# autonomousvision/unimatch

Measured on NVIDIA H100. Metric: image-pairs/sec @480x832 gmflow-scale2-refine6; EPE vs reference, higher is better.
Workload: dtype fp32

## Files before the change

unimatch_b200/csrc/um_conv_tc.cu:

```cuda
#include <stdlib.h>

#include "um_common.cuh"
#include "um_tc.cuh"

namespace um {

using namespace tc;

namespace {

constexpr int TW = 16, TH = 8;
__host__ __device__ constexpr int stages_for(int bn) { return bn >= 96 ? 2 : 3; }
constexpr int NTHREADS = 288;
constexpr int PRODUCER = 8;
constexpr uint32_t A_BYTES = 2 * 16384;
constexpr uint32_t STAGING_UNIT = 16384;
constexpr uint32_t STAGING_BYTES = 2 * STAGING_UNIT;
constexpr uint32_t TAIL_BYTES = 256 + 2048;
__host__ __device__ constexpr uint32_t acc_bytes(int bn) { return (bn < 32 ? 32 : bn) * 128 * 4; }
__host__ __device__ constexpr uint32_t conv_smem_bytes(int bn) {
  return stages_for(bn) * (A_BYTES + 2 * bn * 128) + acc_bytes(bn) + STAGING_BYTES + TAIL_BYTES;
}

struct ConvParams {
  int B, H, W, tiles_x, tiles_y;
  int nsrc, cin_p[2];
  int KH, KW, PH, PW, stride;
  int cout, cout_p;
  const float* bias;
  int mode, act;
  float* out_f32; long long ld_f32; int off_f32;
  __half* out_split; int cp_split, off_split; long long plane_split;
  const float* aux0; long long ld_aux0;
  const float* aux1; long long ld_aux1;
  const float* gamma; const float* beta;
  const float* pre; long long ld_pre;
  int ntiles, tiles_n;
  __half* win_dst; long long win_plane;
  int win_c0, win_c1, win_lp;
  long long win_tokens, win_L;
  Geom win_g;
};

__device__ __forceinline__ float sigmoid_fast(float y) { return __fdividef(1.0f, 1.0f + __expf(-y)); }
__device__ __forceinline__ float tanh_fast(float y) { return 1.0f - __fdividef(2.0f, 1.0f + __expf(2.0f * y)); }
__device__ __forceinline__ uint32_t pack_h2(__half a, __half b) {
  return (uint32_t)__half_as_ushort(a) | ((uint32_t)__half_as_ushort(b) << 16);
}

__device__ __forceinline__ void load_acc32(const float* accs, int r, int c0, float* v) {
  const float* row = accs + (c0 >> 5) * 4096 + r * 32;
#pragma unroll
  for (int i = 0; i < 8; ++i) {
    const float4 x = *reinterpret_cast<const float4*>(row + ((i ^ (r & 7)) << 2));
    v[4 * i] = x.x; v[4 * i + 1] = x.y; v[4 * i + 2] = x.z; v[4 * i + 3] = x.w;
  }
}

template <int BN, int G, int MODE, int ACT, bool WIN = false>
__global__ void __launch_bounds__(NTHREADS, 1)
conv_tc_kernel(const __grid_constant__ CUtensorMap map_a0, const __grid_constant__ CUtensorMap map_a1,
               const __grid_constant__ CUtensorMap map_w, const __grid_constant__ CUtensorMap map_of,
               const __grid_constant__ CUtensorMap map_os, ConvParams p) {
  static_assert(BN == 16 || BN == 64 || BN == 96 || BN == 128, "tile widths 16, 64, 96, 128");
  constexpr int NSB = 1;
  constexpr uint32_t B_BYTES = 2 * BN * 128;
  constexpr uint32_t STAGE_BYTES = A_BYTES + B_BYTES;
  constexpr int STAGES = stages_for(BN);
  constexpr uint32_t ACC_BYTES = acc_bytes(BN);
  extern __shared__ __align__(1024) uint8_t smem[];
  float* accs = reinterpret_cast<float*>(smem + STAGES * STAGE_BYTES);
  float* stage_buf = reinterpret_cast<float*>(smem + STAGES * STAGE_BYTES + ACC_BYTES);
  uint64_t* bars = reinterpret_cast<uint64_t*>(smem + STAGES * STAGE_BYTES + ACC_BYTES + STAGING_BYTES);
  uint64_t* full = bars;
  uint64_t* empty = bars + STAGES;
  float* coef = reinterpret_cast<float*>(reinterpret_cast<uint8_t*>(bars) + 256);
  const int mode = MODE >= 0 ? MODE : p.mode;
  const int act = ACT >= 0 ? ACT : p.act;

  const int warp = threadIdx.x >> 5, lane = threadIdx.x & 31;
  const int taps = p.KH * p.KW;
  int nk = 0;
  for (int s = 0; s < p.nsrc; ++s) nk += taps * (p.cin_p[s] >> 6);

  const int cid = (int)blockIdx.x;
  const int ncid = (int)gridDim.x;

  if (threadIdx.x == 0) {
    for (int i = 0; i < STAGES; ++i) { mbar_init(full + i, 1); mbar_init(empty + i, 8); }
    fence_barrier_init();
  }
  if (warp == PRODUCER && lane == 0) {
    tma_prefetch_desc(&map_a0); tma_prefetch_desc(&map_w);
    if (p.nsrc > 1) tma_prefetch_desc(&map_a1);
  }
  __syncthreads();

  if (warp == PRODUCER) {
    int it = 0;
    for (int t = cid; t < p.ntiles; t += ncid) {
      const int n0 = (t % p.tiles_n) * BN;
      int tile = t / p.tiles_n;
      const int x0 = (tile % p.tiles_x) * TW; tile /= p.tiles_x;
      const int y0 = (tile % p.tiles_y) * TH;
      const int b = tile / p.tiles_y;
      const int chunks0 = p.cin_p[0] >> 6;
      const int nk0 = taps * chunks0;
      const int rot = (int)((unsigned)cid % (unsigned)nk);
      for (int kk = 0; kk < nk; ++kk, ++it) {
        int k = kk + rot; if (k >= nk) k -= nk;
        const int sidx = (k >= nk0) ? 1 : 0;
        const int kl = sidx ? k - nk0 : k;
        const int chunks = sidx ? (p.cin_p[1] >> 6) : chunks0;
        const int tap = kl / chunks, kc = kl - tap * chunks;
        const int ky = tap / p.KW, kx = tap - ky * p.KW;
        const CUtensorMap* ma = sidx ? &map_a1 : &map_a0;
        const int st = it % STAGES;
        mbar_wait_inline(empty + st, ((it / STAGES) & 1) ^ 1);
        uint8_t* sa = smem + st * STAGE_BYTES;
        uint8_t* sb = sa + A_BYTES;
        const int kcol = (sidx ? taps * p.cin_p[0] : 0) + tap * p.cin_p[sidx] + kc * 64;
        if (elect_one()) {
          mbar_arrive_expect_tx(full + st, STAGE_BYTES);
#pragma unroll
          for (int part = 0; part < 2; ++part) {
            tma_load_4d(sa + part * 16384, ma, full + st, kc * 64, x0 * p.stride + kx - p.PW, y0 * p.stride + ky - p.PH, part * p.B + b);
            tma_load_2d(sb + part * (BN * 128), &map_w, full + st, kcol, part * p.cout_p + n0);
          }
        }
        __syncwarp();
      }
    }
  } else {
    const int quarter = warp & 3;
    const int grp = warp >> 2;
    const int r = quarter * 32 + lane;
    const int eg = (warp & 3) * 32 + lane;
    const int frow = grp * 64 + quarter * 16 + (lane >> 2);
    const int fcol = 2 * (lane & 3);
    const bool leader = eg == 0;
    int sctr = 0;
    auto group_sync = [&]() { asm volatile("bar.sync %0, 128;" ::"r"(1 + grp) : "memory"); };
    auto all_sync = [&]() { asm volatile("bar.sync 3, 256;" ::: "memory"); };
    if (mode == UM_CONV_LN && grp == 0) { coef[256 + eg] = __ldg(p.gamma + eg); coef[384 + eg] = __ldg(p.beta + eg); }
    int lt = 0, it = 0;
    for (int t = cid; t < p.ntiles; t += ncid, ++lt) {
      float acc[BN / 2], part[BN / 2];
      for (int k = 0; k < nk; ++k, ++it) {
        const int st = it % STAGES;
        mbar_wait_inline(full + st, (it / STAGES) & 1);
        const uint32_t a_base = smem_u32(smem + st * STAGE_BYTES) + grp * 8192;
        const uint32_t b_base = smem_u32(smem + st * STAGE_BYTES) + A_BYTES;
        const int pa[3] = {1, 0, 0}, pb[3] = {0, 1, 0};
        if (G > 1) fence_acc(part); else fence_acc(acc);
        wgmma_fence();
#pragma unroll
        for (int c = 0; c < 3; ++c)
#pragma unroll
          for (int ks = 0; ks < 4; ++ks) {
            const uint64_t da = desc_kmajor(a_base + pa[c] * 16384 + ks * 32);
            const uint64_t db = desc_kmajor(b_base + pb[c] * (BN * 128) + ks * 32);
            if (G > 1) wgmma_ss<BN>(part, da, db, (c | ks) != 0);
            else wgmma_ss<BN>(acc, da, db, k > 0 || (c | ks) != 0);
          }
        wgmma_commit();
        wgmma_wait<0>();
        if (G > 1) fence_acc(part); else fence_acc(acc);
        __syncwarp();
        if (lane == 0) mbar_arrive(empty + st);
        if (G > 1) {
#pragma unroll
          for (int i = 0; i < BN / 2; ++i) acc[i] = k ? acc[i] + part[i] : part[i];
        }
      }
      all_sync();
#pragma unroll
      for (int j = 0; j < BN / 8; ++j) {
        const int col = 8 * j + fcol;
        float* chunk = accs + (col >> 5) * 4096;
#pragma unroll
        for (int h = 0; h < 2; ++h) {
          const int row = frow + 8 * h;
          *reinterpret_cast<float2*>(chunk + row * 32 + ((((col & 31) >> 2) ^ (row & 7)) << 2) + (col & 3)) =
              make_float2(acc[4 * j + 2 * h], acc[4 * j + 2 * h + 1]);
        }
      }
      all_sync();

      const int n0 = (t % p.tiles_n) * BN;
      int tile = t / p.tiles_n;
      const int x0 = (tile % p.tiles_x) * TW; tile /= p.tiles_x;
      const int y0 = (tile % p.tiles_y) * TH;
      const int b = tile / p.tiles_y;
      const long long pix_r = ((long long)b * p.H + (y0 + (r >> 4))) * p.W + x0 + (r & 15);
      const bool valid_r = (y0 + (r >> 4) < p.H) && (x0 + (r & 15) < p.W);

      auto emit = [&](const float (&v)[32], int co_out, bool to_f32, bool to_split, bool to_win = false) {
        if (WIN && to_win) {
          uint8_t* sbs = reinterpret_cast<uint8_t*>(stage_buf + (grp * NSB + sctr % NSB) * 4096);
          ++sctr;
          if (leader) bulk_wait_read<NSB - 1>();
          group_sync();
#pragma unroll
          for (int i = 0; i < 4; ++i) {
            uint32_t hw[4], lw[4];
#pragma unroll
            for (int e = 0; e < 4; ++e) split_f16x2(v[8 * i + 2 * e], v[8 * i + 2 * e + 1], &hw[e], &lw[e]);
            const int off = r * 64 + ((i ^ ((r >> 1) & 3)) << 4);
            *reinterpret_cast<uint4*>(sbs + off) = make_uint4(hw[0], hw[1], hw[2], hw[3]);
            *reinterpret_cast<uint4*>(sbs + 8192 + off) = make_uint4(lw[0], lw[1], lw[2], lw[3]);
          }
          group_sync();
          const int wc = co_out - p.win_c0;
          __half* obase = p.win_dst + (long long)(wc >> 7) * 2 * p.win_plane + (wc & 127);
          const int* rowdst = reinterpret_cast<const int*>(coef + 256) + (lt & 1) * 128;
          const int piece = eg & 3;
#pragma unroll
          for (int itr = 0; itr < 4; ++itr) {
            const int row = itr * 32 + (eg >> 2);
            const int drow = rowdst[row];
            if (drow < 0) continue;
            const int soff = row * 64 + ((piece ^ ((row >> 1) & 3)) << 4);
            const uint4 hv = *reinterpret_cast<const uint4*>(sbs + soff);
            const uint4 lv = *reinterpret_cast<const uint4*>(sbs + 8192 + soff);
            __half* d = obase + (long long)drow * 128 + piece * 8;
            *reinterpret_cast<uint4*>(d) = hv;
            *reinterpret_cast<uint4*>(d + p.win_plane) = lv;
          }
          return;
        }
        if (to_f32) {
          float* my_stage = stage_buf + (grp * NSB + sctr % NSB) * 4096;
          ++sctr;
          if (leader) bulk_wait_read<NSB - 1>();
          group_sync();
#pragma unroll
          for (int i = 0; i < 8; ++i)
            *reinterpret_cast<float4*>(my_stage + r * 32 + ((i ^ (r & 7)) << 2)) = make_float4(v[4 * i], v[4 * i + 1], v[4 * i + 2], v[4 * i + 3]);
          fence_proxy_async();
          group_sync();
          if (leader) { tma_store_4d(&map_of, my_stage, co_out, x0, y0, b); bulk_commit(); }
        }
        if (to_split) {
          uint8_t* sbs = reinterpret_cast<uint8_t*>(stage_buf + (grp * NSB + sctr % NSB) * 4096);
          ++sctr;
          if (leader) bulk_wait_read<NSB - 1>();
          group_sync();
#pragma unroll
          for (int i = 0; i < 4; ++i) {
            uint32_t hw[4], lw[4];
#pragma unroll
            for (int e = 0; e < 4; ++e) split_f16x2(v[8 * i + 2 * e], v[8 * i + 2 * e + 1], &hw[e], &lw[e]);
            const int off = r * 64 + ((i ^ ((r >> 1) & 3)) << 4);
            *reinterpret_cast<uint4*>(sbs + off) = make_uint4(hw[0], hw[1], hw[2], hw[3]);
            *reinterpret_cast<uint4*>(sbs + 8192 + off) = make_uint4(lw[0], lw[1], lw[2], lw[3]);
          }
          fence_proxy_async();
          group_sync();
          if (leader) {
            tma_store_4d(&map_os, sbs, co_out, x0, y0, b);
            tma_store_4d(&map_os, sbs + 8192, co_out, x0, y0, p.B + b);
            bulk_commit();
          }
        }
      };

      if constexpr (BN == 128) {
        if (mode == UM_CONV_LN) {
          const int ca = grp * 32, cb = 64 + grp * 32;
          float a0[32], a1[32];
          const bool need_a = valid_r && p.aux0;
          if (need_a) {
            const float4* pa = reinterpret_cast<const float4*>(p.aux0 + pix_r * p.ld_aux0 + ca);
            const float4* pb = reinterpret_cast<const float4*>(p.aux0 + pix_r * p.ld_aux0 + cb);
#pragma unroll
            for (int i = 0; i < 8; ++i) {
              const float4 t4 = __ldg(pa + i), u4 = __ldg(pb + i);
              a0[4 * i] = t4.x; a0[4 * i + 1] = t4.y; a0[4 * i + 2] = t4.z; a0[4 * i + 3] = t4.w;
              a1[4 * i] = u4.x; a1[4 * i + 1] = u4.y; a1[4 * i + 2] = u4.z; a1[4 * i + 3] = u4.w;
            }
          }
          float v0[32], v1[32];
          load_acc32(accs, r, ca, v0);
          load_acc32(accs, r, cb, v1);
          float* xs = coef;
          float sum = 0.f;
#pragma unroll
          for (int i = 0; i < 32; ++i) sum += v0[i];
#pragma unroll
          for (int i = 0; i < 32; ++i) sum += v1[i];
          xs[grp * 128 + r] = sum;
          all_sync();
          const float mean = (xs[r] + xs[128 + r]) * (1.0f / 128.0f);
          all_sync();
          float sq = 0.f;
#pragma unroll
          for (int i = 0; i < 32; ++i) { const float dd = v0[i] - mean; sq = fmaf(dd, dd, sq); }
#pragma unroll
          for (int i = 0; i < 32; ++i) { const float dd = v1[i] - mean; sq = fmaf(dd, dd, sq); }
          xs[grp * 128 + r] = sq;
          all_sync();
          const float rstd = rsqrtf((xs[r] + xs[128 + r]) * (1.0f / 128.0f) + 1e-5f);
          const float4* g4a = reinterpret_cast<const float4*>(coef + 256 + ca);
          const float4* b4a = reinterpret_cast<const float4*>(coef + 384 + ca);
          const float4* g4b = reinterpret_cast<const float4*>(coef + 256 + cb);
          const float4* b4b = reinterpret_cast<const float4*>(coef + 384 + cb);
#pragma unroll
          for (int i = 0; i < 8; ++i) {
            const float4 ga = g4a[i], ba = b4a[i], gb = g4b[i], bb = b4b[i];
            v0[4 * i] = (v0[4 * i] - mean) * rstd * ga.x + ba.x;             v1[4 * i] = (v1[4 * i] - mean) * rstd * gb.x + bb.x;
            v0[4 * i + 1] = (v0[4 * i + 1] - mean) * rstd * ga.y + ba.y;     v1[4 * i + 1] = (v1[4 * i + 1] - mean) * rstd * gb.y + bb.y;
            v0[4 * i + 2] = (v0[4 * i + 2] - mean) * rstd * ga.z + ba.z;     v1[4 * i + 2] = (v1[4 * i + 2] - mean) * rstd * gb.z + bb.z;
            v0[4 * i + 3] = (v0[4 * i + 3] - mean) * rstd * ga.w + ba.w;     v1[4 * i + 3] = (v1[4 * i + 3] - mean) * rstd * gb.w + bb.w;
          }
          if (need_a) {
#pragma unroll
            for (int i = 0; i < 32; ++i) { v0[i] += a0[i]; v1[i] += a1[i]; }
          }
          emit(v0, ca, p.out_f32 != nullptr, p.out_split != nullptr);
          emit(v1, cb, p.out_f32 != nullptr, p.out_split != nullptr);
          continue;
        }
      }

      float* sbias = coef + (lt & 1) * 128;
      if (grp == 0) {
        for (int i = eg; i < BN; i += 128) sbias[i] = (p.bias && n0 + i < p.cout) ? __ldg(p.bias + n0 + i) : 0.f;
        if (WIN) {
          const int yy = y0 + (eg >> 4), xx = x0 + (eg & 15);
          const long long token = ((long long)b * p.H + yy) * p.W + xx;
          int drow = -1;
          if (yy < p.H && xx < p.W && token < p.win_tokens) {
            const Geom& g = p.win_g;
            const int n = (int)(token / p.win_L);
            const int t = (int)(token - (long long)n * p.win_L);
            const int ty = t / g.w, tx = t - ty * g.w;
            int yr = ty - g.sh; if (yr < 0) yr += g.h;
            int xr = tx - g.sw; if (xr < 0) xr += g.w;
            const int wy = yr / g.wh, wx = xr / g.ww;
            drow = (n * g.nwin + wy * g.kw + wx) * p.win_lp + (yr - wy * g.wh) * g.ww + (xr - wx * g.ww);
          }
          reinterpret_cast<int*>(coef + 256)[(lt & 1) * 128 + eg] = drow;
        }
      }
      all_sync();
      if (grp * 32 >= BN) continue;

      constexpr int CH = BN < 32 ? BN : 32;
#pragma unroll 1
      for (int c0 = grp * 32; c0 < BN; c0 += 64) {
        const int co0 = n0 + c0;
        const bool live = co0 < p.cout;
        bool to_f32 = p.out_f32 != nullptr, to_split = p.out_split != nullptr;
        int co_out = co0;
        if (mode == UM_CONV_GRU_ZR) {
          to_f32 = co0 < 128; to_split = co0 >= 128;
          if (co0 >= 128) co_out = co0 - 128;
        }
        bool to_win = false;
        if (WIN && co0 >= p.win_c0 && co0 < p.win_c1) { to_win = true; to_f32 = to_split = false; }
        float ax[32], bx[32];
        const bool need_a = live && valid_r && p.aux0 && (mode == UM_CONV_GRU_Q || (mode == UM_CONV_GRU_ZR && co0 >= 128));
        const bool need_b = live && valid_r && mode == UM_CONV_GRU_Q;
        if (need_a) {
          const float4* ap = reinterpret_cast<const float4*>(p.aux0 + pix_r * p.ld_aux0 + (mode == UM_CONV_GRU_ZR ? co0 - 128 : co0));
#pragma unroll
          for (int i = 0; i < 8; ++i) { const float4 t4 = __ldg(ap + i); ax[4 * i] = t4.x; ax[4 * i + 1] = t4.y; ax[4 * i + 2] = t4.z; ax[4 * i + 3] = t4.w; }
        }
        if (need_b) {
          const float4* bp = reinterpret_cast<const float4*>(p.aux1 + pix_r * p.ld_aux1 + co0);
#pragma unroll
          for (int i = 0; i < 8; ++i) { const float4 t4 = __ldg(bp + i); bx[4 * i] = t4.x; bx[4 * i + 1] = t4.y; bx[4 * i + 2] = t4.z; bx[4 * i + 3] = t4.w; }
        }
        float px[32];
        const bool need_p = live && valid_r && p.pre;
        if (need_p) {
          const float4* pp = reinterpret_cast<const float4*>(p.pre + pix_r * p.ld_pre + co0);
#pragma unroll
          for (int i = 0; i < 8; ++i) { const float4 t4 = __ldg(pp + i); px[4 * i] = t4.x; px[4 * i + 1] = t4.y; px[4 * i + 2] = t4.z; px[4 * i + 3] = t4.w; }
        }
        float v[32];
        load_acc32(accs, r, c0, v);
        if (!live) continue;
        if (p.bias) {
          const float4* s4 = reinterpret_cast<const float4*>(sbias + c0);
#pragma unroll
          for (int i = 0; i < CH / 4; ++i) {
            const float4 bb = s4[i];
            v[4 * i] += bb.x; v[4 * i + 1] += bb.y; v[4 * i + 2] += bb.z; v[4 * i + 3] += bb.w;
          }
        }
        if (need_p) {
#pragma unroll
          for (int i = 0; i < CH; ++i) v[i] += px[i];
        }
        if (mode == UM_CONV_GRU_ZR) {
#pragma unroll
          for (int i = 0; i < CH; ++i) v[i] = sigmoid_fast(v[i]);
          if (need_a) {
#pragma unroll
            for (int i = 0; i < CH; ++i) v[i] *= ax[i];
          }
        } else if (mode == UM_CONV_GRU_Q) {
          if (need_b) {
#pragma unroll
            for (int i = 0; i < CH; ++i) v[i] = (1.0f - bx[i]) * ax[i] + bx[i] * tanh_fast(v[i]);
          }
        } else if (act == UM_ACT_RELU) {
#pragma unroll
          for (int i = 0; i < CH; ++i) v[i] = fmaxf(v[i], 0.f);
        } else if (act == UM_ACT_TANH) {
#pragma unroll
          for (int i = 0; i < CH; ++i) v[i] = tanh_fast(v[i]);
        } else if (act == UM_ACT_SIGMOID) {
#pragma unroll
          for (int i = 0; i < CH; ++i) v[i] = sigmoid_fast(v[i]);
        } else if (act == UM_ACT_GELU) {
#pragma unroll
          for (int i = 0; i < CH; ++i) v[i] = act_gelu(v[i]);
        }
        if constexpr (BN >= 32) {
          emit(v, co_out, to_f32, to_split, to_win);
        } else {
          const int nvalid = min(CH, p.cout - co0);
          float* sb = stage_buf + grp * NSB * 4096;
          group_sync();
#pragma unroll
          for (int i = 0; i < CH / 4; ++i)
            *reinterpret_cast<float4*>(sb + r * 32 + ((i ^ (r & 7)) << 2)) = make_float4(v[4 * i], v[4 * i + 1], v[4 * i + 2], v[4 * i + 3]);
          group_sync();
          if (to_f32) {
#pragma unroll 1
            for (int itr = 0; itr < 8; ++itr) {
              const int row = itr * 16 + (eg >> 3), piece = eg & 7;
              const int yy = y0 + (row >> 4), xx = x0 + (row & 15);
              if (yy >= p.H || xx >= p.W || piece * 4 >= nvalid) continue;
              const float4 val = *reinterpret_cast<const float4*>(sb + row * 32 + ((piece ^ (row & 7)) << 2));
              float* dst = p.out_f32 + (((long long)b * p.H + yy) * p.W + xx) * p.ld_f32 + p.off_f32 + co_out + piece * 4;
              const float e[4] = {val.x, val.y, val.z, val.w};
              for (int k = 0; k < 4; ++k) if (piece * 4 + k < nvalid) dst[k] = e[k];
            }
          }
          if (to_split) {
#pragma unroll 1
            for (int itr = 0; itr < 4; ++itr) {
              const int row = itr * 32 + (eg >> 2), piece = eg & 3;
              const int yy = y0 + (row >> 4), xx = x0 + (row & 15);
              if (yy >= p.H || xx >= p.W || piece * 8 >= nvalid) continue;
              const float4 a4 = *reinterpret_cast<const float4*>(sb + row * 32 + (((2 * piece) ^ (row & 7)) << 2));
              const float4 c4 = *reinterpret_cast<const float4*>(sb + row * 32 + (((2 * piece + 1) ^ (row & 7)) << 2));
              const float e[8] = {a4.x, a4.y, a4.z, a4.w, c4.x, c4.y, c4.z, c4.w};
              __half* dh = p.out_split + (((long long)b * p.H + yy) * p.W + xx) * p.cp_split + p.off_split + co_out + piece * 8;
              __half* dl = dh + p.plane_split;
              for (int k = 0; k < 8; ++k)
                if (piece * 8 + k < nvalid) { __half h0, l0; split_f16(e[k], &h0, &l0); dh[k] = h0; dl[k] = l0; }
            }
          }
        }
      }
    }
    if (leader) bulk_wait_all();
  }
}

template <int VEC>
__global__ void __launch_bounds__(256) split_planes_kernel(const float* __restrict__ src, long long ld, int C,
                                                           __half* __restrict__ dst, int cp, int off, long long plane,
                                                           long long rows) {
  const int per_row = C / VEC;
  const long long i = (long long)blockIdx.x * blockDim.x + threadIdx.x;
  if (i >= rows * per_row) return;
  const long long row = i / per_row;
  const int c = (int)(i - row * per_row) * VEC;
  if (VEC == 4) {
    const float4 x = __ldg(reinterpret_cast<const float4*>(src + row * ld + c));
    __half h[4], l[4];
    split_f16(x.x, &h[0], &l[0]); split_f16(x.y, &h[1], &l[1]); split_f16(x.z, &h[2], &l[2]); split_f16(x.w, &h[3], &l[3]);
    *reinterpret_cast<uint2*>(dst + row * cp + off + c) = make_uint2(pack_h2(h[0], h[1]), pack_h2(h[2], h[3]));
    *reinterpret_cast<uint2*>(dst + plane + row * cp + off + c) = make_uint2(pack_h2(l[0], l[1]), pack_h2(l[2], l[3]));
  } else {
    __half h, l;
    split_f16(__ldg(src + row * ld + c), &h, &l);
    dst[row * cp + off + c] = h;
    dst[plane + row * cp + off + c] = l;
  }
}

}

int make_map_4d_f16(CUtensorMap* map, const void* base, uint64_t cp, uint64_t W, uint64_t H, uint64_t NB, uint32_t stride,
                    uint64_t plane_elems) {
  PFN_encodeTiled enc = get_encode_tiled();
  if (!enc) { set_error("cuTensorMapEncodeTiled unavailable"); return UM_ECUDA; }
  cuuint64_t dims[4] = {cp, W, H, NB};
  cuuint64_t strides[3] = {cp * 2, cp * W * 2, (plane_elems ? plane_elems : cp * W * H) * 2};
  cuuint32_t box[4] = {64, 16 * stride, 8 * stride, 1};
  cuuint32_t estr[4] = {1, stride, stride, 1};
  CUresult r = enc(map, CU_TENSOR_MAP_DATA_TYPE_FLOAT16, 4, const_cast<void*>(base), dims, strides, box, estr,
                   CU_TENSOR_MAP_INTERLEAVE_NONE, CU_TENSOR_MAP_SWIZZLE_128B, CU_TENSOR_MAP_L2_PROMOTION_L2_128B,
                   CU_TENSOR_MAP_FLOAT_OOB_FILL_NONE);
  if (r != CUDA_SUCCESS) { set_error("cuTensorMapEncodeTiled(4d) failed (%d)", (int)r); return UM_ECUDA; }
  return UM_OK;
}

int make_map_out(CUtensorMap* map, void* base, int elem_bytes, uint64_t cout, uint64_t ld, uint64_t W, uint64_t H, uint64_t N,
                 uint64_t plane_elems) {
  PFN_encodeTiled enc = get_encode_tiled();
  if (!enc) { set_error("cuTensorMapEncodeTiled unavailable"); return UM_ECUDA; }
  cuuint64_t dims[4] = {cout, W, H, N};
  cuuint64_t strides[3] = {ld * elem_bytes, ld * W * elem_bytes, (plane_elems ? plane_elems : ld * W * H) * elem_bytes};
  cuuint32_t box[4] = {32, 16, 8, 1};
  cuuint32_t estr[4] = {1, 1, 1, 1};
  CUresult r = enc(map, elem_bytes == 4 ? CU_TENSOR_MAP_DATA_TYPE_FLOAT32 : CU_TENSOR_MAP_DATA_TYPE_FLOAT16, 4, base, dims,
                   strides, box, estr, CU_TENSOR_MAP_INTERLEAVE_NONE,
                   elem_bytes == 4 ? CU_TENSOR_MAP_SWIZZLE_128B : CU_TENSOR_MAP_SWIZZLE_64B,
                   CU_TENSOR_MAP_L2_PROMOTION_NONE, CU_TENSOR_MAP_FLOAT_OOB_FILL_NONE);
  if (r != CUDA_SUCCESS) { set_error("cuTensorMapEncodeTiled(out) failed (%d)", (int)r); return UM_ECUDA; }
  return UM_OK;
}

namespace {

template <int BN, int G, int MODE, int ACT, bool WIN = false>
int launch_conv(const CUtensorMap& m0, const CUtensorMap& m1, const CUtensorMap& mw, const CUtensorMap& mof,
                const CUtensorMap& mos, const ConvParams& p, cudaStream_t st) {
  constexpr uint32_t smem = conv_smem_bytes(BN);
  static_assert(smem <= 232448, "shared memory budget");
  static PerDeviceBytes configured;
  if (int rc = ensure_smem(configured, conv_tc_kernel<BN, G, MODE, ACT, WIN>, smem, "conv_tc")) return rc;
// ... 161 lines not shown
```

unimatch_b200/csrc/um_tc.cuh:

```cuda
#pragma once
#include <cuda.h>
#include <cuda_fp16.h>
#include <cuda_runtime.h>
#include <stdint.h>

namespace um {
namespace tc {

__device__ __forceinline__ uint32_t smem_u32(const void* p) { return (uint32_t)__cvta_generic_to_shared(p); }

__device__ __forceinline__ bool elect_one() {
  uint32_t pred = 0;
  asm volatile(
      "{\n\t.reg .pred P;\n\telect.sync _|P, 0xffffffff;\n\tselp.u32 %0, 1, 0, P;\n\t}\n"
      : "=r"(pred));
  return pred != 0;
}

__device__ __forceinline__ void mbar_init(uint64_t* bar, uint32_t count) {
  asm volatile("mbarrier.init.shared::cta.b64 [%0], %1;" ::"r"(smem_u32(bar)), "r"(count));
}
__device__ __forceinline__ void fence_barrier_init() { asm volatile("fence.mbarrier_init.release.cluster;" ::: "memory"); }
__device__ __forceinline__ void fence_proxy_async() { asm volatile("fence.proxy.async.shared::cta;" ::: "memory"); }
__device__ __forceinline__ void mbar_arrive(uint64_t* bar) {
  asm volatile("mbarrier.arrive.shared::cta.b64 _, [%0];" ::"r"(smem_u32(bar)) : "memory");
}
__device__ __forceinline__ void mbar_arrive_expect_tx(uint64_t* bar, uint32_t bytes) {
  asm volatile("mbarrier.arrive.expect_tx.shared::cta.b64 _, [%0], %1;" ::"r"(smem_u32(bar)), "r"(bytes) : "memory");
}
__device__ __forceinline__ bool mbar_try_wait(uint64_t* bar, uint32_t parity) {
  uint32_t ok;
  asm volatile(
      "{\n\t.reg .pred P;\n\tmbarrier.try_wait.parity.shared::cta.b64 P, [%1], %2;\n\tselp.u32 %0, 1, 0, P;\n\t}\n"
      : "=r"(ok)
      : "r"(smem_u32(bar)), "r"(parity)
      : "memory");
  return ok != 0;
}
static __device__ __noinline__ void mbar_wait_slow(uint64_t* bar, uint32_t parity) {
#pragma unroll 1
  for (uint32_t i = 0; i < (1u << 22); ++i)
    if (mbar_try_wait(bar, parity)) return;
  printf("um::tc mbarrier timeout: block (%d,%d,%d) thread %d bar %p parity %u\n", blockIdx.x, blockIdx.y, blockIdx.z,
         threadIdx.x, (void*)bar, parity);
  __trap();
}
__device__ __forceinline__ void mbar_wait(uint64_t* bar, uint32_t parity) {
  if (!mbar_try_wait(bar, parity)) mbar_wait_slow(bar, parity);
}
__device__ __forceinline__ void mbar_wait_inline(uint64_t* bar, uint32_t parity) {
#pragma unroll 1
  for (uint32_t i = 0; !mbar_try_wait(bar, parity); ++i)
    if (i == (1u << 22)) __trap();
}

__device__ __forceinline__ void tma_prefetch_desc(const CUtensorMap* m) {
  asm volatile("prefetch.tensormap [%0];" ::"l"(reinterpret_cast<uint64_t>(m)) : "memory");
}
__device__ __forceinline__ void tma_load_2d(void* dst, const CUtensorMap* m, uint64_t* bar, int c0, int c1) {
  asm volatile(
      "cp.async.bulk.tensor.2d.shared::cluster.global.mbarrier::complete_tx::bytes [%0], [%1, {%3, %4}], [%2];"
      ::"r"(smem_u32(dst)), "l"(reinterpret_cast<uint64_t>(m)), "r"(smem_u32(bar)), "r"(c0), "r"(c1)
      : "memory");
}
__device__ __forceinline__ void tma_load_4d(void* dst, const CUtensorMap* m, uint64_t* bar, int c0, int c1, int c2, int c3) {
  asm volatile(
      "cp.async.bulk.tensor.4d.shared::cluster.global.mbarrier::complete_tx::bytes [%0], [%1, {%3, %4, %5, %6}], [%2];"
      ::"r"(smem_u32(dst)), "l"(reinterpret_cast<uint64_t>(m)), "r"(smem_u32(bar)), "r"(c0), "r"(c1), "r"(c2), "r"(c3)
      : "memory");
}

__device__ __forceinline__ void tma_store_4d(const CUtensorMap* m, const void* src, int c0, int c1, int c2, int c3) {
  asm volatile("cp.async.bulk.tensor.4d.global.shared::cta.bulk_group [%0, {%2, %3, %4, %5}], [%1];"
               ::"l"(reinterpret_cast<uint64_t>(m)), "r"(smem_u32(src)), "r"(c0), "r"(c1), "r"(c2), "r"(c3)
               : "memory");
}
__device__ __forceinline__ void bulk_commit() { asm volatile("cp.async.bulk.commit_group;" ::: "memory"); }
template <int N>
__device__ __forceinline__ void bulk_wait_read() { asm volatile("cp.async.bulk.wait_group.read %0;" ::"n"(N) : "memory"); }
__device__ __forceinline__ void bulk_wait_all() { asm volatile("cp.async.bulk.wait_group 0;" ::: "memory"); }

__device__ __forceinline__ uint64_t smem_desc_sw128(uint32_t saddr, uint32_t lbo_bytes, uint32_t sbo_bytes) {
  uint64_t d = 0;
  d |= (uint64_t)((saddr & 0x3FFFF) >> 4);
  d |= (uint64_t)((lbo_bytes >> 4) & 0x3FFF) << 16;
  d |= (uint64_t)((sbo_bytes >> 4) & 0x3FFF) << 32;
  d |= (uint64_t)1 << 62;
  return d;
}
__device__ __forceinline__ uint64_t desc_kmajor(uint32_t saddr) { return smem_desc_sw128(saddr, 16, 1024); }
__device__ __forceinline__ uint64_t desc_mnmajor(uint32_t saddr, uint32_t mn_group_stride) {
  return smem_desc_sw128(saddr, mn_group_stride, 1024);
}

__device__ __forceinline__ void wgmma_fence() { asm volatile("wgmma.fence.sync.aligned;" ::: "memory"); }
__device__ __forceinline__ void wgmma_commit() { asm volatile("wgmma.commit_group.sync.aligned;" ::: "memory"); }
template <int N>
__device__ __forceinline__ void wgmma_wait() { asm volatile("wgmma.wait_group.sync.aligned %0;" ::"n"(N) : "memory"); }
template <int N>
__device__ __forceinline__ void fence_acc(float (&d)[N]) {
#pragma unroll
  for (int i = 0; i < N; ++i) asm volatile("" : "+f"(d[i])::"memory");
}

template <int N>
__device__ __forceinline__ void wgmma_ss(float (&d)[N / 2], uint64_t da, uint64_t db, bool accumulate);
template <>
__device__ __forceinline__ void wgmma_ss<16>(float (&d)[8], uint64_t da, uint64_t db, bool accumulate) {
  asm volatile(
      "{\n\t.reg .pred p;\n\tsetp.ne.b32 p, %10, 0;\n\t"
      "wgmma.mma_async.sync.aligned.m64n16k16.f32.f16.f16 {%0, %1, %2, %3, %4, %5, %6, %7}, %8, %9, p, 1, 1, 0, 0;\n\t}\n"
      : "+f"(d[0]), "+f"(d[1]), "+f"(d[2]), "+f"(d[3]), "+f"(d[4]), "+f"(d[5]), "+f"(d[6]), "+f"(d[7])
      : "l"(da), "l"(db), "r"((uint32_t)accumulate));
}
template <>
__device__ __forceinline__ void wgmma_ss<64>(float (&d)[32], uint64_t da, uint64_t db, bool accumulate) {
  asm volatile(
      "{\n\t.reg .pred p;\n\tsetp.ne.b32 p, %34, 0;\n\t"
      "wgmma.mma_async.sync.aligned.m64n64k16.f32.f16.f16 {%0, %1, %2, %3, %4, %5, %6, %7, %8, %9, %10, %11, %12, %13, %14, %15, %16, %17, %18, %19, %20, %21, %22, %23, %24, %25, %26, %27, %28, %29, %30, %31}, %32, %33, p, 1, 1, 0, 0;\n\t}\n"
      : "+f"(d[0]), "+f"(d[1]), "+f"(d[2]), "+f"(d[3]), "+f"(d[4]), "+f"(d[5]), "+f"(d[6]), "+f"(d[7]), "+f"(d[8]), "+f"(d[9]), "+f"(d[10]), "+f"(d[11]), "+f"(d[12]), "+f"(d[13]), "+f"(d[14]), "+f"(d[15]), "+f"(d[16]), "+f"(d[17]), "+f"(d[18]), "+f"(d[19]), "+f"(d[20]), "+f"(d[21]), "+f"(d[22]), "+f"(d[23]), "+f"(d[24]), "+f"(d[25]), "+f"(d[26]), "+f"(d[27]), "+f"(d[28]), "+f"(d[29]), "+f"(d[30]), "+f"(d[31])
      : "l"(da), "l"(db), "r"((uint32_t)accumulate));
}
template <>
__device__ __forceinline__ void wgmma_ss<96>(float (&d)[48], uint64_t da, uint64_t db, bool accumulate) {
  asm volatile(
      "{\n\t.reg .pred p;\n\tsetp.ne.b32 p, %50, 0;\n\t"
      "wgmma.mma_async.sync.aligned.m64n96k16.f32.f16.f16 {%0, %1, %2, %3, %4, %5, %6, %7, %8, %9, %10, %11, %12, %13, %14, %15, %16, %17, %18, %19, %20, %21, %22, %23, %24, %25, %26, %27, %28, %29, %30, %31, %32, %33, %34, %35, %36, %37, %38, %39, %40, %41, %42, %43, %44, %45, %46, %47}, %48, %49, p, 1, 1, 0, 0;\n\t}\n"
      : "+f"(d[0]), "+f"(d[1]), "+f"(d[2]), "+f"(d[3]), "+f"(d[4]), "+f"(d[5]), "+f"(d[6]), "+f"(d[7]), "+f"(d[8]), "+f"(d[9]), "+f"(d[10]), "+f"(d[11]), "+f"(d[12]), "+f"(d[13]), "+f"(d[14]), "+f"(d[15]), "+f"(d[16]), "+f"(d[17]), "+f"(d[18]), "+f"(d[19]), "+f"(d[20]), "+f"(d[21]), "+f"(d[22]), "+f"(d[23]), "+f"(d[24]), "+f"(d[25]), "+f"(d[26]), "+f"(d[27]), "+f"(d[28]), "+f"(d[29]), "+f"(d[30]), "+f"(d[31]), "+f"(d[32]), "+f"(d[33]), "+f"(d[34]), "+f"(d[35]), "+f"(d[36]), "+f"(d[37]), "+f"(d[38]), "+f"(d[39]), "+f"(d[40]), "+f"(d[41]), "+f"(d[42]), "+f"(d[43]), "+f"(d[44]), "+f"(d[45]), "+f"(d[46]), "+f"(d[47])
      : "l"(da), "l"(db), "r"((uint32_t)accumulate));
}
template <>
__device__ __forceinline__ void wgmma_ss<128>(float (&d)[64], uint64_t da, uint64_t db, bool accumulate) {
  asm volatile(
      "{\n\t.reg .pred p;\n\tsetp.ne.b32 p, %66, 0;\n\t"
      "wgmma.mma_async.sync.aligned.m64n128k16.f32.f16.f16 {%0, %1, %2, %3, %4, %5, %6, %7, %8, %9, %10, %11, %12, %13, %14, %15, %16, %17, %18, %19, %20, %21, %22, %23, %24, %25, %26, %27, %28, %29, %30, %31, %32, %33, %34, %35, %36, %37, %38, %39, %40, %41, %42, %43, %44, %45, %46, %47, %48, %49, %50, %51, %52, %53, %54, %55, %56, %57, %58, %59, %60, %61, %62, %63}, %64, %65, p, 1, 1, 0, 0;\n\t}\n"
      : "+f"(d[0]), "+f"(d[1]), "+f"(d[2]), "+f"(d[3]), "+f"(d[4]), "+f"(d[5]), "+f"(d[6]), "+f"(d[7]), "+f"(d[8]), "+f"(d[9]), "+f"(d[10]), "+f"(d[11]), "+f"(d[12]), "+f"(d[13]), "+f"(d[14]), "+f"(d[15]), "+f"(d[16]), "+f"(d[17]), "+f"(d[18]), "+f"(d[19]), "+f"(d[20]), "+f"(d[21]), "+f"(d[22]), "+f"(d[23]), "+f"(d[24]), "+f"(d[25]), "+f"(d[26]), "+f"(d[27]), "+f"(d[28]), "+f"(d[29]), "+f"(d[30]), "+f"(d[31]), "+f"(d[32]), "+f"(d[33]), "+f"(d[34]), "+f"(d[35]), "+f"(d[36]), "+f"(d[37]), "+f"(d[38]), "+f"(d[39]), "+f"(d[40]), "+f"(d[41]), "+f"(d[42]), "+f"(d[43]), "+f"(d[44]), "+f"(d[45]), "+f"(d[46]), "+f"(d[47]), "+f"(d[48]), "+f"(d[49]), "+f"(d[50]), "+f"(d[51]), "+f"(d[52]), "+f"(d[53]), "+f"(d[54]), "+f"(d[55]), "+f"(d[56]), "+f"(d[57]), "+f"(d[58]), "+f"(d[59]), "+f"(d[60]), "+f"(d[61]), "+f"(d[62]), "+f"(d[63])
      : "l"(da), "l"(db), "r"((uint32_t)accumulate));
}
__device__ __forceinline__ void wgmma_rs_n128_tb(float (&d)[64], const uint32_t (&a)[4], uint64_t db, bool accumulate) {
  asm volatile(
      "{\n\t.reg .pred p;\n\tsetp.ne.b32 p, %69, 0;\n\t"
      "wgmma.mma_async.sync.aligned.m64n128k16.f32.f16.f16 {%0, %1, %2, %3, %4, %5, %6, %7, %8, %9, %10, %11, %12, %13, %14, %15, %16, %17, %18, %19, %20, %21, %22, %23, %24, %25, %26, %27, %28, %29, %30, %31, %32, %33, %34, %35, %36, %37, %38, %39, %40, %41, %42, %43, %44, %45, %46, %47, %48, %49, %50, %51, %52, %53, %54, %55, %56, %57, %58, %59, %60, %61, %62, %63}, {%64, %65, %66, %67}, %68, p, 1, 1, 1;\n\t}\n"
      : "+f"(d[0]), "+f"(d[1]), "+f"(d[2]), "+f"(d[3]), "+f"(d[4]), "+f"(d[5]), "+f"(d[6]), "+f"(d[7]), "+f"(d[8]), "+f"(d[9]), "+f"(d[10]), "+f"(d[11]), "+f"(d[12]), "+f"(d[13]), "+f"(d[14]), "+f"(d[15]), "+f"(d[16]), "+f"(d[17]), "+f"(d[18]), "+f"(d[19]), "+f"(d[20]), "+f"(d[21]), "+f"(d[22]), "+f"(d[23]), "+f"(d[24]), "+f"(d[25]), "+f"(d[26]), "+f"(d[27]), "+f"(d[28]), "+f"(d[29]), "+f"(d[30]), "+f"(d[31]), "+f"(d[32]), "+f"(d[33]), "+f"(d[34]), "+f"(d[35]), "+f"(d[36]), "+f"(d[37]), "+f"(d[38]), "+f"(d[39]), "+f"(d[40]), "+f"(d[41]), "+f"(d[42]), "+f"(d[43]), "+f"(d[44]), "+f"(d[45]), "+f"(d[46]), "+f"(d[47]), "+f"(d[48]), "+f"(d[49]), "+f"(d[50]), "+f"(d[51]), "+f"(d[52]), "+f"(d[53]), "+f"(d[54]), "+f"(d[55]), "+f"(d[56]), "+f"(d[57]), "+f"(d[58]), "+f"(d[59]), "+f"(d[60]), "+f"(d[61]), "+f"(d[62]), "+f"(d[63])
      : "r"(a[0]), "r"(a[1]), "r"(a[2]), "r"(a[3]), "l"(db), "r"((uint32_t)accumulate));
}

__device__ __forceinline__ void wgmma_rs_n64(float (&d)[32], const uint32_t (&a)[4], uint64_t db, bool accumulate) {
  asm volatile(
      "{\n\t.reg .pred p;\n\tsetp.ne.b32 p, %37, 0;\n\t"
      "wgmma.mma_async.sync.aligned.m64n64k16.f32.f16.f16 {%0, %1, %2, %3, %4, %5, %6, %7, %8, %9, %10, %11, %12, %13, %14, %15, %16, %17, %18, %19, %20, %21, %22, %23, %24, %25, %26, %27, %28, %29, %30, %31}, {%32, %33, %34, %35}, %36, p, 1, 1, 0;\n\t}\n"
      : "+f"(d[0]), "+f"(d[1]), "+f"(d[2]), "+f"(d[3]), "+f"(d[4]), "+f"(d[5]), "+f"(d[6]), "+f"(d[7]), "+f"(d[8]), "+f"(d[9]), "+f"(d[10]), "+f"(d[11]), "+f"(d[12]), "+f"(d[13]), "+f"(d[14]), "+f"(d[15]), "+f"(d[16]), "+f"(d[17]), "+f"(d[18]), "+f"(d[19]), "+f"(d[20]), "+f"(d[21]), "+f"(d[22]), "+f"(d[23]), "+f"(d[24]), "+f"(d[25]), "+f"(d[26]), "+f"(d[27]), "+f"(d[28]), "+f"(d[29]), "+f"(d[30]), "+f"(d[31])
      : "r"(a[0]), "r"(a[1]), "r"(a[2]), "r"(a[3]), "l"(db), "r"((uint32_t)accumulate));
}

__device__ __forceinline__ void split_f16(float x, __half* hi, __half* lo) {
  const __half h = __float2half_rn(x);
  *hi = h;
  *lo = __float2half_rn(x - __half2float(h));
}

__device__ __forceinline__ void split_f16x2(float a, float b, uint32_t* hi, uint32_t* lo) {
  const __half2 h = __floats2half2_rn(a, b);
  const float2 hf = __half22float2(h);
  const __half2 l = __floats2half2_rn(a - hf.x, b - hf.y);
  *hi = *reinterpret_cast<const uint32_t*>(&h);
  *lo = *reinterpret_cast<const uint32_t*>(&l);
}
__device__ __forceinline__ float ex2_approx(float x) {
  float y;
  asm("ex2.approx.ftz.f32 %0, %1;" : "=f"(y) : "f"(x));
  return y;
}

__device__ __forceinline__ float act_gelu(float y) {
  const float a = fminf(fabsf(y), 8.5f);
  float q = 3.151970304e-06f;
// ... 29 lines not shown
```

Measured before the change: 54.50.

## Split conv epilogue into dedicated warpgroup overlapping with MMA via mbarriers

```diff
diff --git a/unimatch_b200/csrc/um_conv_tc.cu b/unimatch_b200/csrc/um_conv_tc.cu
--- a/unimatch_b200/csrc/um_conv_tc.cu
+++ b/unimatch_b200/csrc/um_conv_tc.cu
@@ -11,8 +11,10 @@
 
 constexpr int TW = 16, TH = 8;
 __host__ __device__ constexpr int stages_for(int bn) { return bn >= 96 ? 2 : 3; }
-constexpr int NTHREADS = 288;
-constexpr int PRODUCER = 8;
+constexpr int NTHREADS = 512;
+constexpr int EPILOGUE = 8;
+constexpr int PRODUCER = 12;
+constexpr int REGS_PRODUCER = 32, REGS_MMA = 168, REGS_EPI = 144;
 constexpr uint32_t A_BYTES = 2 * 16384;
 constexpr uint32_t STAGING_UNIT = 16384;
 constexpr uint32_t STAGING_BYTES = 2 * STAGING_UNIT;
@@ -63,7 +65,7 @@
                const __grid_constant__ CUtensorMap map_w, const __grid_constant__ CUtensorMap map_of,
                const __grid_constant__ CUtensorMap map_os, ConvParams p) {
   static_assert(BN == 16 || BN == 64 || BN == 96 || BN == 128, "tile widths 16, 64, 96, 128");
-  constexpr int NSB = 1;
+  constexpr int NSB = 2;
   constexpr uint32_t B_BYTES = 2 * BN * 128;
   constexpr uint32_t STAGE_BYTES = A_BYTES + B_BYTES;
   constexpr int STAGES = stages_for(BN);
@@ -74,20 +76,23 @@
   uint64_t* bars = reinterpret_cast<uint64_t*>(smem + STAGES * STAGE_BYTES + ACC_BYTES + STAGING_BYTES);
   uint64_t* full = bars;
   uint64_t* empty = bars + STAGES;
+  uint64_t* acc_full = bars + 2 * STAGES;
+  uint64_t* acc_empty = acc_full + 1;
   float* coef = reinterpret_cast<float*>(reinterpret_cast<uint8_t*>(bars) + 256);
   const int mode = MODE >= 0 ? MODE : p.mode;
   const int act = ACT >= 0 ? ACT : p.act;
 
   const int warp = threadIdx.x >> 5, lane = threadIdx.x & 31;
-  const int taps = p.KH * p.KW;
-  int nk = 0;
-  for (int s = 0; s < p.nsrc; ++s) nk += taps * (p.cin_p[s] >> 6);
-
-  const int cid = (int)blockIdx.x;
-  const int ncid = (int)gridDim.x;
+  auto k_stages = [&]() {
+    int n = 0;
+    for (int s = 0; s < p.nsrc; ++s) n += p.KH * p.KW * (p.cin_p[s] >> 6);
+    return n;
+  };
 
   if (threadIdx.x == 0) {
     for (int i = 0; i < STAGES; ++i) { mbar_init(full + i, 1); mbar_init(empty + i, 8); }
+    mbar_init(acc_full, 256);
+    mbar_init(acc_empty, 128);
     fence_barrier_init();
   }
   if (warp == PRODUCER && lane == 0) {
@@ -96,7 +101,12 @@
   }
   __syncthreads();
 
-  if (warp == PRODUCER) {
+  if (warp >= PRODUCER) {
+    setmaxnreg_dec<REGS_PRODUCER>();
+    if (warp != PRODUCER) return;
+    const int cid = (int)blockIdx.x, ncid = (int)gridDim.x;
+    const int taps = p.KH * p.KW;
+    const int nk = k_stages();
     int it = 0;
     for (int t = cid; t < p.ntiles; t += ncid) {
       const int n0 = (t % p.tiles_n) * BN;
@@ -131,18 +141,14 @@
         __syncwarp();
       }
     }
-  } else {
+  } else if (warp < EPILOGUE) {
+    setmaxnreg_inc<REGS_MMA>();
+    const int cid = (int)blockIdx.x, ncid = (int)gridDim.x;
+    const int nk = k_stages();
     const int quarter = warp & 3;
     const int grp = warp >> 2;
-    const int r = quarter * 32 + lane;
-    const int eg = (warp & 3) * 32 + lane;
     const int frow = grp * 64 + quarter * 16 + (lane >> 2);
     const int fcol = 2 * (lane & 3);
-    const bool leader = eg == 0;
-    int sctr = 0;
-    auto group_sync = [&]() { asm volatile("bar.sync %0, 128;" ::"r"(1 + grp) : "memory"); };
-    auto all_sync = [&]() { asm volatile("bar.sync 3, 256;" ::: "memory"); };
-    if (mode == UM_CONV_LN && grp == 0) { coef[256 + eg] = __ldg(p.gamma + eg); coef[384 + eg] = __ldg(p.beta + eg); }
     int lt = 0, it = 0;
     for (int t = cid; t < p.ntiles; t += ncid, ++lt) {
       float acc[BN / 2], part[BN / 2];
@@ -173,7 +179,7 @@
           for (int i = 0; i < BN / 2; ++i) acc[i] = k ? acc[i] + part[i] : part[i];
         }
       }
-      all_sync();
+      mbar_wait_inline(acc_empty, (lt & 1) ^ 1);
 #pragma unroll
       for (int j = 0; j < BN / 8; ++j) {
         const int col = 8 * j + fcol;
@@ -185,8 +191,19 @@
               make_float2(acc[4 * j + 2 * h], acc[4 * j + 2 * h + 1]);
         }
       }
-      all_sync();
-
+      mbar_arrive(acc_full);
+    }
+  } else {
+    setmaxnreg_inc<REGS_EPI>();
+    const int cid = (int)blockIdx.x, ncid = (int)gridDim.x;
+    const int r = threadIdx.x - EPILOGUE * 32;
+    const bool leader = r == 0;
+    int sctr = 0;
+    auto epi_sync = [&]() { asm volatile("bar.sync 1, 128;" ::: "memory"); };
+    if (mode == UM_CONV_LN) { coef[256 + r] = __ldg(p.gamma + r); coef[384 + r] = __ldg(p.beta + r); }
+    epi_sync();
+    int lt = 0;
+    for (int t = cid; t < p.ntiles; t += ncid, ++lt) {
       const int n0 = (t % p.tiles_n) * BN;
       int tile = t / p.tiles_n;
       const int x0 = (tile % p.tiles_x) * TW; tile /= p.tiles_x;
@@ -197,10 +214,10 @@
 
       auto emit = [&](const float (&v)[32], int co_out, bool to_f32, bool to_split, bool to_win = false) {
         if (WIN && to_win) {
-          uint8_t* sbs = reinterpret_cast<uint8_t*>(stage_buf + (grp * NSB + sctr % NSB) * 4096);
+          uint8_t* sbs = reinterpret_cast<uint8_t*>(stage_buf + (sctr % NSB) * 4096);
           ++sctr;
-          if (leader) bulk_wait_read<NSB - 1>();
-          group_sync();
+          if (leader) bulk_wait_read<0>();
+          epi_sync();
 #pragma unroll
           for (int i = 0; i < 4; ++i) {
             uint32_t hw[4], lw[4];
@@ -210,14 +227,14 @@
             *reinterpret_cast<uint4*>(sbs + off) = make_uint4(hw[0], hw[1], hw[2], hw[3]);
             *reinterpret_cast<uint4*>(sbs + 8192 + off) = make_uint4(lw[0], lw[1], lw[2], lw[3]);
           }
-          group_sync();
+          epi_sync();
           const int wc = co_out - p.win_c0;
           __half* obase = p.win_dst + (long long)(wc >> 7) * 2 * p.win_plane + (wc & 127);
           const int* rowdst = reinterpret_cast<const int*>(coef + 256) + (lt & 1) * 128;
-          const int piece = eg & 3;
+          const int piece = r & 3;
 #pragma unroll
           for (int itr = 0; itr < 4; ++itr) {
-            const int row = itr * 32 + (eg >> 2);
+            const int row = itr * 32 + (r >> 2);
             const int drow = rowdst[row];
             if (drow < 0) continue;
             const int soff = row * 64 + ((piece ^ ((row >> 1) & 3)) << 4);
@@ -230,22 +247,22 @@
           return;
         }
         if (to_f32) {
-          float* my_stage = stage_buf + (grp * NSB + sctr % NSB) * 4096;
+          float* my_stage = stage_buf + (sctr % NSB) * 4096;
           ++sctr;
           if (leader) bulk_wait_read<NSB - 1>();
-          group_sync();
+          epi_sync();
 #pragma unroll
           for (int i = 0; i < 8; ++i)
             *reinterpret_cast<float4*>(my_stage + r * 32 + ((i ^ (r & 7)) << 2)) = make_float4(v[4 * i], v[4 * i + 1], v[4 * i + 2], v[4 * i + 3]);
           fence_proxy_async();
-          group_sync();
+          epi_sync();
           if (leader) { tma_store_4d(&map_of, my_stage, co_out, x0, y0, b); bulk_commit(); }
         }
         if (to_split) {
-          uint8_t* sbs = reinterpret_cast<uint8_t*>(stage_buf + (grp * NSB + sctr % NSB) * 4096);
+          uint8_t* sbs = reinterpret_cast<uint8_t*>(stage_buf + (sctr % NSB) * 4096);
           ++sctr;
           if (leader) bulk_wait_read<NSB - 1>();
-          group_sync();
+          epi_sync();
 #pragma unroll
           for (int i = 0; i < 4; ++i) {
             uint32_t hw[4], lw[4];
@@ -256,7 +273,7 @@
             *reinterpret_cast<uint4*>(sbs + 8192 + off) = make_uint4(lw[0], lw[1], lw[2], lw[3]);
           }
           fence_proxy_async();
-          group_sync();
+          epi_sync();
           if (leader) {
             tma_store_4d(&map_os, sbs, co_out, x0, y0, b);
             tma_store_4d(&map_os, sbs + 8192, co_out, x0, y0, p.B + b);
@@ -267,88 +284,89 @@
 
       if constexpr (BN == 128) {
         if (mode == UM_CONV_LN) {
-          const int ca = grp * 32, cb = 64 + grp * 32;
-          float a0[32], a1[32];
+          mbar_wait_inline(acc_full, lt & 1);
+          float sum0 = 0.f, sum1 = 0.f, sq0 = 0.f, sq1 = 0.f;
+#pragma unroll 1
+          for (int h = 0; h < 2; ++h) {
+            float v0[32], v1[32];
+            load_acc32(accs, r, 32 * h, v0);
+            load_acc32(accs, r, 64 + 32 * h, v1);
+            float sum = 0.f;
+#pragma unroll
+            for (int i = 0; i < 32; ++i) sum += v0[i];
+#pragma unroll
+            for (int i = 0; i < 32; ++i) sum += v1[i];
+            if (h == 0) sum0 = sum; else sum1 = sum;
+          }
+          const float mean = (sum0 + sum1) * (1.0f / 128.0f);
+#pragma unroll 1
+          for (int h = 0; h < 2; ++h) {
+            float v0[32], v1[32];
+            load_acc32(accs, r, 32 * h, v0);
+            load_acc32(accs, r, 64 + 32 * h, v1);
+            float sq = 0.f;
+#pragma unroll
+            for (int i = 0; i < 32; ++i) { const float dd = v0[i] - mean; sq = fmaf(dd, dd, sq); }
+#pragma unroll
+            for (int i = 0; i < 32; ++i) { const float dd = v1[i] - mean; sq = fmaf(dd, dd, sq); }
+            if (h == 0) sq0 = sq; else sq1 = sq;
+          }
+          const float rstd = rsqrtf((sq0 + sq1) * (1.0f / 128.0f) + 1e-5f);
           const bool need_a = valid_r && p.aux0;
-          if (need_a) {
-            const float4* pa = reinterpret_cast<const float4*>(p.aux0 + pix_r * p.ld_aux0 + ca);
-            const float4* pb = reinterpret_cast<const float4*>(p.aux0 + pix_r * p.ld_aux0 + cb);
+#pragma unroll 1
+          for (int c0 = 0; c0 < 128; c0 += 32) {
+            float a[32];
+            if (need_a) {
+              const float4* pa = reinterpret_cast<const float4*>(p.aux0 + pix_r * p.ld_aux0 + c0);
+#pragma unroll
+              for (int i = 0; i < 8; ++i) { const float4 t4 = __ldg(pa + i); a[4 * i] = t4.x; a[4 * i + 1] = t4.y; a[4 * i + 2] = t4.z; a[4 * i + 3] = t4.w; }
+            }
+            float v[32];
+            load_acc32(accs, r, c0, v);
+            if (c0 == 96) mbar_arrive(acc_empty);
+            const float4* g4 = reinterpret_cast<const float4*>(coef + 256 + c0);
+            const float4* b4 = reinterpret_cast<const float4*>(coef + 384 + c0);
 #pragma unroll
             for (int i = 0; i < 8; ++i) {
-              const float4 t4 = __ldg(pa + i), u4 = __ldg(pb + i);
-              a0[4 * i] = t4.x; a0[4 * i + 1] = t4.y; a0[4 * i + 2] = t4.z; a0[4 * i + 3] = t4.w;
-              a1[4 * i] = u4.x; a1[4 * i + 1] = u4.y; a1[4 * i + 2] = u4.z; a1[4 * i + 3] = u4.w;
+              const float4 g = g4[i], bb = b4[i];
+              v[4 * i] = (v[4 * i] - mean) * rstd * g.x + bb.x;
+              v[4 * i + 1] = (v[4 * i + 1] - mean) * rstd * g.y + bb.y;
+              v[4 * i + 2] = (v[4 * i + 2] - mean) * rstd * g.z + bb.z;
+              v[4 * i + 3] = (v[4 * i + 3] - mean) * rstd * g.w + bb.w;
             }
-          }
-          float v0[32], v1[32];
-          load_acc32(accs, r, ca, v0);
-          load_acc32(accs, r, cb, v1);
-          float* xs = coef;
-          float sum = 0.f;
-#pragma unroll
-          for (int i = 0; i < 32; ++i) sum += v0[i];
-#pragma unroll
-          for (int i = 0; i < 32; ++i) sum += v1[i];
-          xs[grp * 128 + r] = sum;
-          all_sync();
-          const float mean = (xs[r] + xs[128 + r]) * (1.0f / 128.0f);
-          all_sync();
-          float sq = 0.f;
-#pragma unroll
-          for (int i = 0; i < 32; ++i) { const float dd = v0[i] - mean; sq = fmaf(dd, dd, sq); }
-#pragma unroll
-          for (int i = 0; i < 32; ++i) { const float dd = v1[i] - mean; sq = fmaf(dd, dd, sq); }
-          xs[grp * 128 + r] = sq;
-          all_sync();
-          const float rstd = rsqrtf((xs[r] + xs[128 + r]) * (1.0f / 128.0f) + 1e-5f);
-          const float4* g4a = reinterpret_cast<const float4*>(coef + 256 + ca);
-          const float4* b4a = reinterpret_cast<const float4*>(coef + 384 + ca);
-          const float4* g4b = reinterpret_cast<const float4*>(coef + 256 + cb);
-          const float4* b4b = reinterpret_cast<const float4*>(coef + 384 + cb);
-#pragma unroll
-          for (int i = 0; i < 8; ++i) {
-            const float4 ga = g4a[i], ba = b4a[i], gb = g4b[i], bb = b4b[i];
-            v0[4 * i] = (v0[4 * i] - mean) * rstd * ga.x + ba.x;             v1[4 * i] = (v1[4 * i] - mean) * rstd * gb.x + bb.x;
-            v0[4 * i + 1] = (v0[4 * i + 1] - mean) * rstd * ga.y + ba.y;     v1[4 * i + 1] = (v1[4 * i + 1] - mean) * rstd * gb.y + bb.y;
-            v0[4 * i + 2] = (v0[4 * i + 2] - mean) * rstd * ga.z + ba.z;     v1[4 * i + 2] = (v1[4 * i + 2] - mean) * rstd * gb.z + bb.z;
-            v0[4 * i + 3] = (v0[4 * i + 3] - mean) * rstd * ga.w + ba.w;     v1[4 * i + 3] = (v1[4 * i + 3] - mean) * rstd * gb.w + bb.w;
-          }
-          if (need_a) {
-#pragma unroll
-            for (int i = 0; i < 32; ++i) { v0[i] += a0[i]; v1[i] += a1[i]; }
-          }
-          emit(v0, ca, p.out_f32 != nullptr, p.out_split != nullptr);
-          emit(v1, cb, p.out_f32 != nullptr, p.out_split != nullptr);
+            if (need_a) {
+#pragma unroll
+              for (int i = 0; i < 32; ++i) v[i] += a[i];
+            }
+            emit(v, c0, p.out_f32 != nullptr, p.out_split != nullptr);
+          }
           continue;
         }
       }
 
       float* sbias = coef + (lt & 1) * 128;
-      if (grp == 0) {
-        for (int i = eg; i < BN; i += 128) sbias[i] = (p.bias && n0 + i < p.cout) ? __ldg(p.bias + n0 + i) : 0.f;
-        if (WIN) {
-          const int yy = y0 + (eg >> 4), xx = x0 + (eg & 15);
-          const long long token = ((long long)b * p.H + yy) * p.W + xx;
-          int drow = -1;
-          if (yy < p.H && xx < p.W && token < p.win_tokens) {
-            const Geom& g = p.win_g;
-            const int n = (int)(token / p.win_L);
-            const int t = (int)(token - (long long)n * p.win_L);
-            const int ty = t / g.w, tx = t - ty * g.w;
-            int yr = ty - g.sh; if (yr < 0) yr += g.h;
-            int xr = tx - g.sw; if (xr < 0) xr += g.w;
-            const int wy = yr / g.wh, wx = xr / g.ww;
-            drow = (n * g.nwin + wy * g.kw + wx) * p.win_lp + (yr - wy * g.wh) * g.ww + (xr - wx * g.ww);
-          }
-          reinterpret_cast<int*>(coef + 256)[(lt & 1) * 128 + eg] = drow;
-        }
+      if (r < BN) sbias[r] = (p.bias && n0 + r < p.cout) ? __ldg(p.bias + n0 + r) : 0.f;
+      if (WIN) {
+        const int yy = y0 + (r >> 4), xx = x0 + (r & 15);
+        const long long token = ((long long)b * p.H + yy) * p.W + xx;
+        int drow = -1;
+        if (yy < p.H && xx < p.W && token < p.win_tokens) {
+          const Geom& g = p.win_g;
+          const int n = (int)(token / p.win_L);
+          const int t = (int)(token - (long long)n * p.win_L);
+          const int ty = t / g.w, tx = t - ty * g.w;
+          int yr = ty - g.sh; if (yr < 0) yr += g.h;
+          int xr = tx - g.sw; if (xr < 0) xr += g.w;
+          const int wy = yr / g.wh, wx = xr / g.ww;
+          drow = (n * g.nwin + wy * g.kw + wx) * p.win_lp + (yr - wy * g.wh) * g.ww + (xr - wx * g.ww);
+        }
+        reinterpret_cast<int*>(coef + 256)[(lt & 1) * 128 + r] = drow;
       }
-      all_sync();
-      if (grp * 32 >= BN) continue;
+      epi_sync();
 
       constexpr int CH = BN < 32 ? BN : 32;
 #pragma unroll 1
-      for (int c0 = grp * 32; c0 < BN; c0 += 64) {
+      for (int c0 = 0; c0 < BN; c0 += 32) {
         const int co0 = n0 + c0;
         const bool live = co0 < p.cout;
         bool to_f32 = p.out_f32 != nullptr, to_split = p.out_split != nullptr;
@@ -359,19 +377,6 @@
         }
         bool to_win = false;
         if (WIN && co0 >= p.win_c0 && co0 < p.win_c1) { to_win = true; to_f32 = to_split = false; }
-        float ax[32], bx[32];
-        const bool need_a = live && valid_r && p.aux0 && (mode == UM_CONV_GRU_Q || (mode == UM_CONV_GRU_ZR && co0 >= 128));
-        const bool need_b = live && valid_r && mode == UM_CONV_GRU_Q;
-        if (need_a) {
-          const float4* ap = reinterpret_cast<const float4*>(p.aux0 + pix_r * p.ld_aux0 + (mode == UM_CONV_GRU_ZR ? co0 - 128 : co0));
-#pragma unroll
-          for (int i = 0; i < 8; ++i) { const float4 t4 = __ldg(ap + i); ax[4 * i] = t4.x; ax[4 * i + 1] = t4.y; ax[4 * i + 2] = t4.z; ax[4 * i + 3] = t4.w; }
-        }
-        if (need_b) {
-          const float4* bp = reinterpret_cast<const float4*>(p.aux1 + pix_r * p.ld_aux1 + co0);
-#pragma unroll
-          for (int i = 0; i < 8; ++i) { const float4 t4 = __ldg(bp + i); bx[4 * i] = t4.x; bx[4 * i + 1] = t4.y; bx[4 * i + 2] = t4.z; bx[4 * i + 3] = t4.w; }
-        }
         float px[32];
         const bool need_p = live && valid_r && p.pre;
         if (need_p) {
@@ -380,7 +385,9 @@
           for (int i = 0; i < 8; ++i) { const float4 t4 = __ldg(pp + i); px[4 * i] = t4.x; px[4 * i + 1] = t4.y; px[4 * i + 2] = t4.z; px[4 * i + 3] = t4.w; }
         }
         float v[32];
+        mbar_wait_inline(acc_full, lt & 1);
         load_acc32(accs, r, c0, v);
+        if (c0 + 32 >= BN) mbar_arrive(acc_empty);
         if (!live) continue;
         if (p.bias) {
           const float4* s4 = reinterpret_cast<const float4*>(sbias + c0);
@@ -393,6 +400,19 @@
         if (need_p) {
 #pragma unroll
           for (int i = 0; i < CH; ++i) v[i] += px[i];
+        }
+        float ax[32], bx[32];
+        const bool need_a = valid_r && p.aux0 && (mode == UM_CONV_GRU_Q || (mode == UM_CONV_GRU_ZR && co0 >= 128));
+        const bool need_b = valid_r && mode == UM_CONV_GRU_Q;
+        if (need_a) {
+          const float4* ap = reinterpret_cast<const float4*>(p.aux0 + pix_r * p.ld_aux0 + (mode == UM_CONV_GRU_ZR ? co0 - 128 : co0));
+#pragma unroll
+          for (int i = 0; i < 8; ++i) { const float4 t4 = __ldg(ap + i); ax[4 * i] = t4.x; ax[4 * i + 1] = t4.y; ax[4 * i + 2] = t4.z; ax[4 * i + 3] = t4.w; }
+        }
+        if (need_b) {
+          const float4* bp = reinterpret_cast<const float4*>(p.aux1 + pix_r * p.ld_aux1 + co0);
+#pragma unroll
+          for (int i = 0; i < 8; ++i) { const float4 t4 = __ldg(bp + i); bx[4 * i] = t4.x; bx[4 * i + 1] = t4.y; bx[4 * i + 2] = t4.z; bx[4 * i + 3] = t4.w; }
         }
         if (mode == UM_CONV_GRU_ZR) {
 #pragma unroll
@@ -423,16 +443,16 @@
           emit(v, co_out, to_f32, to_split, to_win);
         } else {
           const int nvalid = min(CH, p.cout - co0);
-          float* sb = stage_buf + grp * NSB * 4096;
-          group_sync();
+          float* sb = stage_buf;
+          epi_sync();
 #pragma unroll
           for (int i = 0; i < CH / 4; ++i)
             *reinterpret_cast<float4*>(sb + r * 32 + ((i ^ (r & 7)) << 2)) = make_float4(v[4 * i], v[4 * i + 1], v[4 * i + 2], v[4 * i + 3]);
-          group_sync();
+          epi_sync();
           if (to_f32) {
 #pragma unroll 1
             for (int itr = 0; itr < 8; ++itr) {
-              const int row = itr * 16 + (eg >> 3), piece = eg & 7;
+              const int row = itr * 16 + (r >> 3), piece = r & 7;
               const int yy = y0 + (row >> 4), xx = x0 + (row & 15);
               if (yy >= p.H || xx >= p.W || piece * 4 >= nvalid) continue;
               const float4 val = *reinterpret_cast<const float4*>(sb + row * 32 + ((piece ^ (row & 7)) << 2));
@@ -444,7 +464,7 @@
           if (to_split) {
 #pragma unroll 1
             for (int itr = 0; itr < 4; ++itr) {
-              const int row = itr * 32 + (eg >> 2), piece = eg & 3;
+              const int row = itr * 32 + (r >> 2), piece = r & 3;
               const int yy = y0 + (row >> 4), xx = x0 + (row & 15);
               if (yy >= p.H || xx >= p.W || piece * 8 >= nvalid) continue;
               const float4 a4 = *reinterpret_cast<const float4*>(sb + row * 32 + (((2 * piece) ^ (row & 7)) << 2));
diff --git a/unimatch_b200/csrc/um_tc.cuh b/unimatch_b200/csrc/um_tc.cuh
--- a/unimatch_b200/csrc/um_tc.cuh
+++ b/unimatch_b200/csrc/um_tc.cuh
@@ -92,6 +92,11 @@
 __device__ __forceinline__ uint64_t desc_mnmajor(uint32_t saddr, uint32_t mn_group_stride) {
   return smem_desc_sw128(saddr, mn_group_stride, 1024);
 }
+
+template <int N>
+__device__ __forceinline__ void setmaxnreg_inc() { asm volatile("setmaxnreg.inc.sync.aligned.u32 %0;" ::"n"(N)); }
+template <int N>
+__device__ __forceinline__ void setmaxnreg_dec() { asm volatile("setmaxnreg.dec.sync.aligned.u32 %0;" ::"n"(N)); }
 
 __device__ __forceinline__ void wgmma_fence() { asm volatile("wgmma.fence.sync.aligned;" ::: "memory"); }
 __device__ __forceinline__ void wgmma_commit() { asm volatile("wgmma.commit_group.sync.aligned;" ::: "memory"); }
```

After: 64.51, median of 6. 18.4% higher.
